# openxrlab/xrslam

Measured on AMD Instinct MI355X. Metric: frames/sec, full per-frame hot path (KLT tracker + sliding-window VI-BA), one sequence per GPU, higher is better.
Workload: dtype u8/i16 images, f32 LK with exact i64 reductions, f64 BA

## Files before the change

xrslam_amd/csrc/ba_chain.hip.h:

```cpp
#pragma once
#include "ba_kernels.hip.h"

namespace xrhip {

constexpr int CHAIN_MAX_NA = 90;
constexpr int CHAIN_MAX_NI = 8;
constexpr int CHAIN_MAX_F = 64;
constexpr int CHAIN_MAX_OBS = 1024;
constexpr int CHAIN_MAX_FREE = 6;
constexpr int CHAIN_THREADS = 256;

#ifdef XRHIP_KPROF
#define CPROF(slot)                                   \
    do {                                              \
        if (threadIdx.x == 0) {                       \
            const long long cp_n = wall_clock64();    \
            s_ctl.prof[slot] += cp_n - cp_t;          \
            cp_t = cp_n;                              \
        }                                             \
    } while (0)
#else
#define CPROF(slot) \
    do {            \
    } while (0)
#endif

struct ChainLayout {
    int sx, cs, Hp, gp, A, scr, sp, D, gs, grad, gn, delta, gt, wJi, wJj, wr, bref, raw, Hv, oc, rec, xch, total;
};
__host__ __device__ __forceinline__ ChainLayout chain_layout(int F, int na, int NI, int nfree, int nobs) {
    ChainLayout L;
    int o = 0;
    auto take = [&](int n) {
        const int r = o;
        o += (n + 1) & ~1;
        return r;
    };
    L.sx = take(16 * F);
    L.cs = take(16 * F);
    L.Hp = take(na * (na + 1) / 2);
    L.gp = take(na);
    L.A = take(na <= CH_NB ? 2 : tl_doubles(na + 1) + 16 * tl_tile_rows(na + 1));
    L.scr = take(NI * IMU_SCR);
    L.sp = take(na);
    L.D = take(na);
    L.gs = take(na);
    L.grad = take(na);
    L.gn = take(na);
    L.delta = take(na);
    L.gt = take(na);
    L.wJi = take(225 * NI);
    L.wJj = take(225 * NI);
    L.wr = take(16 * NI);
    L.bref = take(6 * NI);
    L.raw = take(15 * NI);
    L.Hv = take(28 * nfree);
    L.oc = take(nobs);
    L.rec = take(XRHIP_IMU_DIM * NI);
    L.xch = take(IMU_XCH * NI);
    L.total = o;
    return L;
}

constexpr int CHAIN_VIS_TILE = 4 * 27 * 65;
constexpr int CHAIN_OBS_CACHE = 16;
enum { CHAIN_OPT_TILE = 1, CHAIN_OPT_CACHE = 2 };
__host__ __device__ __forceinline__ int chain_cache_stride(int M) { return (M + 1) & ~1; }

__device__ __forceinline__ double obs_eval_cached(const BaDims &d, const double *oca, int Mp, int o, const double *state, const Ext &cam,
                                                  double sx, double sy, bool want_j, double *rec, const double *ftab, const int *slot_of,
                                                  const double *ctab) {
    const int inf = (int)oca[15 * Mp + o];
    const int ft = inf & 255, fr = (inf >> 8) & 255;
    const bool at = (inf >> 16) & 1, ar = (inf >> 17) & 1;
    if (!at && !ar) {
        if (want_j)
            for (int i = 0; i < OREC; ++i) rec[i] = 0.0;
        return 0.0;
    }
    ObsConst c;
    c.b1 = v3(oca[o], oca[Mp + o], oca[2 * Mp + o]);
    c.b2 = v3(oca[3 * Mp + o], oca[4 * Mp + o], oca[5 * Mp + o]);
    c.y_ref_center = v3(oca[6 * Mp + o], oca[7 * Mp + o], oca[8 * Mp + o]);
    c.x = v3(oca[9 * Mp + o], oca[10 * Mp + o], oca[11 * Mp + o]);
    const V3 zt = v3(oca[12 * Mp + o], oca[13 * Mp + o], oca[14 * Mp + o]);
    double r[2], Jt[12], Jr[12];
#pragma unroll
    for (int i = 0; i < 12; ++i) Jr[i] = 0.0;
    if (!ar) {
        eval_reprojection_tgt(ftab + 12 * slot_of[ft], ctab, c, zt, sx, sy, r, want_j, Jt);
    } else {
        const FState st = load_state(state + 16 * ft), sr = load_state(state + 16 * fr);
        eval_reprojection_cached(st, sr, ar, c, zt, cam, sx, sy, r, want_j, Jt, Jr);
    }
    const double s = r[0] * r[0] + r[1] * r[1];
    if (want_j) {
        const double sc = d.robust ? sqrt(fmax(2.2250738585072014e-308, 1.0 / (1.0 + s))) : 1.0;
#pragma unroll
        for (int i = 0; i < 12; ++i) {
            rec[i] = at ? Jt[i] * sc : 0.0;
            rec[12 + i] = ar ? Jr[i] * sc : 0.0;
        }
        rec[24] = 0.0;
        rec[25] = 0.0;
        rec[26] = r[0] * sc;
        rec[27] = r[1] * sc;
    }
    return d.robust ? 0.5 * log(1.0 + s) : 0.5 * s;
}

struct ChainArgs {
    const TinyArgs *args;
    int seq, max_rounds, opts;
    const double *link_src;
    int link_frame;
};
__global__ __launch_bounds__(CHAIN_THREADS) void kb_chain(Batch<ChainArgs> batch) {
    const TinyArgs *__restrict__ args = batch.e[blockIdx.z].args;
    const int seq = batch.e[blockIdx.z].seq, max_rounds = batch.e[blockIdx.z].max_rounds, opts = batch.e[blockIdx.z].opts;
    const double *link_src = batch.e[blockIdx.z].link_src;
    const int link_frame = batch.e[blockIdx.z].link_src ? batch.e[blockIdx.z].link_frame : -1;
    const BaDims &d = args->d;
    const BaPtrs &p = args->p;
    const Ext &cam = args->cam, &imu = args->imu;
    const double sx_ = args->sx, sy_ = args->sy;
    extern __shared__ double lds[];
    __shared__ double scratch[64];
    __shared__ double Dblk[CH_NB][CH_NB + 1];
    __shared__ double s_vis[4][CHAIN_MAX_FREE][27];
    __shared__ int s_fail;
    __shared__ int s_free[CHAIN_MAX_FREE], s_slot[CHAIN_MAX_F], s_nfree;
    __shared__ double s_ftab[2][CHAIN_MAX_FREE][12], s_ctab[12];
    __shared__ BaCtl s_ctl;
    const int tid = threadIdx.x, lane = tid & 63;
    const bool split = d.NI > 0;
    const bool imu_lane = lane < d.NI;
    const int ostride = split ? 192 : 256;
    const int otid = (!split || tid < 192) ? tid : (1 << 30);
    const int wtid = tid, wave = tid >> 6;
    constexpr bool worker = true;
    constexpr int nt = 256;
    const int F = d.F, n = d.n, na = d.na, NI = d.NI, M = d.M, MR = d.MR;
#ifdef XRHIP_KPROF
    long long cp_t = wall_clock64();
    const long long cp_t0 = cp_t;
#endif

    if (tid < 64) {
        const bool fr = tid < F && p.fix[tid < F ? tid : 0] != 3;
        const unsigned long long m = __ballot(fr);
        const int slot = __popcll(m & ((1ull << tid) - 1ull));
        if (tid < F) s_slot[tid] = (fr && slot < CHAIN_MAX_FREE) ? slot : -1;
        if (fr && slot < CHAIN_MAX_FREE) s_free[slot] = tid;
        if (tid == 0) s_nfree = min(__popcll(m), CHAIN_MAX_FREE);
    } else {
        constexpr unsigned ctl_words = sizeof(BaCtl) / sizeof(long long);
        const long long *src = reinterpret_cast<const long long *>(static_cast<BaCtl *>(p.ctl));
        long long *dst = reinterpret_cast<long long *>(&s_ctl);
        for (unsigned i = tid - 64; i < ctl_words; i += nt - 64) dst[i] = src[i];
    }
    __syncthreads();
    const int nfree = s_nfree;
    const ChainLayout Lo = chain_layout(F, na, NI, nfree, M + MR);
    double *const X = lds + Lo.sx, *const CS = lds + Lo.cs, *const Hp = lds + Lo.Hp, *const gp = lds + Lo.gp;
    double *const A = lds + Lo.A, *const sp = lds + Lo.sp, *const Dg = lds + Lo.D, *const gs = lds + Lo.gs;
    double *const grad = lds + Lo.grad, *const gn = lds + Lo.gn, *const delta = lds + Lo.delta, *const gt = lds + Lo.gt;
    double *const wJi = lds + Lo.wJi, *const wJj = lds + Lo.wJj, *const wr = lds + Lo.wr, *const bref = lds + Lo.bref;
    double *const raw = lds + Lo.raw, *const Hv = lds + Lo.Hv, *const oc = lds + Lo.oc, *const recs = lds + Lo.rec, *const xch = lds + Lo.xch;
    double *const scr = lds + Lo.scr;
    const bool vis_tile = (opts & CHAIN_OPT_TILE) != 0, use_cache = (opts & CHAIN_OPT_CACHE) != 0;
    const int Mp = chain_cache_stride(M);
    double *const oca = lds + Lo.total + (vis_tile ? CHAIN_VIS_TILE : 0);
    BaCtl *const c = &s_ctl;

    int act[4];
#pragma unroll
    for (int m = 0; m < 4; ++m) {
        const int a = tid + nt * m;
        act[m] = (worker && a < n) ? p.act_inv[a] : -1;
    }
    for (int e = wtid; e < 16 * F; e += nt) X[e] = (e >> 4) == link_frame ? link_src[e & 15] : p.state[e];
    for (int e = wtid; e < 6 * NI; e += nt) bref[e] = p.imu_i[e / 6] == link_frame ? link_src[10 + e % 6] : p.bias_ref[e];
    for (int e = wtid; e < XRHIP_IMU_DIM * NI; e += nt) recs[e] = p.imu_data[e];
    for (int e = wtid; e < NI * IMU_SCR; e += nt) scr[e] = 0.0;
    __syncthreads();
    if (tid < nfree) frame_table(load_state(X + 16 * s_free[tid]), s_ftab[0][tid]);
    else if (tid == 64) ext_table(cam, s_ctab);
    if (use_cache) {
        for (int o = wtid; o < M; o += nt) {
            const int ft = p.obs_tgt[o], fr = p.obs_ref[o];
            const bool at = pose_free(p.fix[ft]), ar = pose_free(p.fix[fr]);
            const V3 zt = v3(p.obs_zt[3 * o], p.obs_zt[3 * o + 1], p.obs_zt[3 * o + 2]);
            if (at || ar) {
                const V3 zr = v3(p.obs_zr[3 * o], p.obs_zr[3 * o + 1], p.obs_zr[3 * o + 2]);
                const ObsConst c = reprojection_constants(load_state(X + 16 * fr), p.depth[p.obs_lm[o]], zt, zr, cam);
                oca[o] = c.b1.x; oca[Mp + o] = c.b1.y; oca[2 * Mp + o] = c.b1.z;
                oca[3 * Mp + o] = c.b2.x; oca[4 * Mp + o] = c.b2.y; oca[5 * Mp + o] = c.b2.z;
                oca[6 * Mp + o] = c.y_ref_center.x; oca[7 * Mp + o] = c.y_ref_center.y; oca[8 * Mp + o] = c.y_ref_center.z;
                oca[9 * Mp + o] = c.x.x; oca[10 * Mp + o] = c.x.y; oca[11 * Mp + o] = c.x.z;
                oca[12 * Mp + o] = zt.x; oca[13 * Mp + o] = zt.y; oca[14 * Mp + o] = zt.z;
            }
            oca[15 * Mp + o] = (double)(ft | (fr << 8) | ((int)at << 16) | ((int)ar << 17));
        }
    }
    __syncthreads();
    CPROF(0);

    bool relin = true;
    int mode = 1, st = ST_RUNNING;
    for (int round = 0; round < max_rounds; ++round) {
        if (relin) {
#ifdef XRHIP_KPROF
            const long long pa_t0 = wall_clock64();
#endif
            for (int o = otid; o < M; o += ostride) {
                double rec[OREC];
                const double co = use_cache ? obs_eval_cached(d, oca, Mp, o, X, cam, sx_, sy_, true, rec, &s_ftab[0][0][0], s_slot, s_ctab)
                                            : obs_eval(d, p, o, X, p.depth, cam, sx_, sy_, true, rec);
                oc[o] = co;
#pragma unroll
                for (int i = 0; i < OREC; ++i) p.orec[(size_t)o * OREC + i] = rec[i];
            }
            for (int o = otid; o < MR; o += ostride) {
                double rec[RREC];
                const double co = rot_eval(d, p, o, X, cam, sx_, sy_, true, rec);
                oc[M + o] = co;
#pragma unroll
                for (int i = 0; i < RREC; ++i) p.rrec[(size_t)o * RREC + i] = rec[i];
            }
#ifdef XRHIP_KPROF
            const long long pa_t1 = wall_clock64();
            if (tid == 0) s_ctl.prof[21] += pa_t1 - pa_t0;
#endif
            bool imu_on = false;
            int nfi = 0, nfj = 0;
            if (imu_lane) {
                const int k = lane, fi = p.imu_i[k], fj = p.imu_j[k];
                nfi = p.fix[fi] != 3;
                nfj = p.fix[fj] != 3;
                imu_on = nfi || nfj;
                if (imu_on) {
                    double *rw = scr + k * IMU_SCR;
                    const FState si = load_state(X + 16 * fi), sj = load_state(X + 16 * fj);
                    const ImuRec pre = load_imu(recs + k * XRHIP_IMU_DIM);
                    const V3 bg0 = v3(bref[6 * k], bref[6 * k + 1], bref[6 * k + 2]);
                    const V3 ba0 = v3(bref[6 * k + 3], bref[6 * k + 4], bref[6 * k + 5]);
                    if (wave == 3) {
                        const V3 rq = imu_residual_rq(si, sj, pre, bg0, imu);
                        rw[0] = rq.x;
                        rw[1] = rq.y;
                        rw[2] = rq.z;
                        double *xk = xch + k * IMU_XCH;
                        store33(xk + 45, imu_jac_jrinv(rq));
                        if (nfi) store33(xk + 36, imu_jac_B(rq));
                        imu_residual_rest(si, sj, pre, bg0, ba0, imu, rw);
                    } else if (wave == 0) {
                        imu_raw_jacobians_part(2, si, sj, pre, bg0, ba0, imu, v3(0, 0, 0), rw + 15, rw + 240, nfi, nfj);
                    } else if (wave == 1) {
                        imu_jac_pre(si, sj, pre, bg0, imu, xch + k * IMU_XCH, nfi, nfj);
                    } else {
                        imu_raw_jacobians_part(3, si, sj, pre, bg0, ba0, imu, v3(0, 0, 0), rw + 15, rw + 240, nfi, nfj);
                    }
                }
            }
#ifdef XRHIP_KPROF
            if (tid == 192) atomicAdd((unsigned long long *)&s_ctl.prof[22], (unsigned long long)(wall_clock64() - pa_t1));
            if (tid == 0) atomicAdd((unsigned long long *)&s_ctl.prof[23], (unsigned long long)(wall_clock64() - pa_t1));
#endif
            __syncthreads();
            CPROF(18);
            auto vis_blocks = [&](int idx, int stride) __attribute__((always_inline)) {
                for (int s = 0; s < nfree; ++s) {
                    const int f = s_free[s], pair = f * F + f;
                    const int s0 = p.pair_start[pair], s1 = p.pair_start[pair + 1];
                    double acc[27];
#pragma unroll
                    for (int i = 0; i < 27; ++i) acc[i] = 0.0;
                    for (int it = s0 + idx; it < s1; it += stride) {
                        const int code = p.pair_items[it];
                        const double *rec = p.orec + (size_t)(code >> 1) * OREC + ((code & 1) ? 12 : 0);
                        double j[12];
#pragma unroll
                        for (int i = 0; i < 12; ++i) j[i] = rec[i];
                        const double *rr = p.orec + (size_t)(code >> 1) * OREC + 26;
                        const double r0 = rr[0], r1 = rr[1];
                        int e = 0;
#pragma unroll
                        for (int a = 0; a < 6; ++a) {
#pragma unroll
                            for (int b = a; b < 6; ++b) acc[e++] += j[a] * j[b] + j[6 + a] * j[6 + b];
                            acc[21 + a] += j[a] * r0 + j[6 + a] * r1;
                        }
                    }
                    if (vis_tile) {
                        double *tw = lds + Lo.total + wave * (27 * 65);
#pragma unroll
                        for (int i = 0; i < 27; ++i) tw[i * 65 + lane] = acc[i];
                        wave_sync();
                        const int row = lane < 27 ? lane : lane - 27;
                        double s2 = 0.0;
                        if (lane < 54) {
                            const double *rp = tw + row * 65 + (lane < 27 ? 0 : 32);
#pragma unroll
                            for (int i = 0; i < 32; ++i) s2 += rp[i];
                        }
                        const double hi = __shfl(s2, (lane + 27) & 63);
                        if (lane < 27) s_vis[wave][s][lane] = s2 + hi;
                        wave_sync();
                    } else {
#pragma unroll
                        for (int i = 0; i < 27; ++i) acc[i] = wave_sum(acc[i]);
                        if (lane == 0)
#pragma unroll
                            for (int i = 0; i < 27; ++i) s_vis[wave][s][i] = acc[i];
                    }
                }
            };
            if (split) {
                if (wave >= 2) {
                    vis_blocks(tid - 128, 128);
                } else if (imu_on) {
                    double *rw = scr + lane * IMU_SCR;
                    const double *xk = xch + lane * IMU_XCH;
                    if (wave == 0) imu_jac_finish0(load33(xk + 45), xk, rw + 15, rw + 240, nfi, nfj);
                    else if (wave == 1)
                        imu_jac_finish1(load33(xk + 45), load33(xk + 36), xk, load33(recs + lane * XRHIP_IMU_DIM + 11), rw + 15, nfi);
                }
            } else {
                vis_blocks(tid, nt);
            }
            __syncthreads();
            CPROF(1);
            for (int e = tid; e < 27 * nfree; e += nt) {
                const int s = e / 27, q = e - 27 * s;
                Hv[28 * s + q] = split ? s_vis[2][s][q] + s_vis[3][s][q] : (s_vis[0][s][q] + s_vis[1][s][q]) + (s_vis[2][s][q] + s_vis[3][s][q]);
            }
            for (int k = 0; k < NI; ++k) {
                const double *rw = scr + k * IMU_SCR, *Ji = rw + 15, *Jj = rw + 240;
                const int fi = p.imu_i[k], fj = p.imu_j[k];
                const bool active = !(p.fix[fi] == 3 && p.fix[fj] == 3);
                const double *S = recs + k * XRHIP_IMU_DIM + 56;
                if (wave == (k & 3)) {
                    double cost = 0.0;
                    if (lane < 15) {
                        double s = 0;
                        if (active)
                            for (int j = 0; j < 15; ++j) s += S[15 * lane + j] * rw[j];
                        wr[16 * k + lane] = s;
                        cost = 0.5 * s * s;
                    }
                    cost = wave_sum(cost);
                    if (lane == 0) wr[16 * k + 15] = cost;
                }
                if (wtid < 225) {
                    const int e = wtid, i = e / 15, cc = e - 15 * i;
                    double a = 0, b = 0;
                    if (active) {
                        const bool col_i = cc < 6 ? pose_free(p.fix[fi]) : motion_free(p.fix[fi]);
                        const bool col_j = cc < 6 ? pose_free(p.fix[fj]) : motion_free(p.fix[fj]);
                        if (col_i)
                            for (int j = 0; j < 15; ++j) a += S[15 * i + j] * Ji[15 * j + cc];
                        if (col_j)
                            for (int j = 0; j < 15; ++j) b += S[15 * i + j] * Jj[15 * j + cc];
                    }
                    wJi[225 * k + e] = a;
                    wJj[225 * k + e] = b;
                }
            }
            __syncthreads();
            CPROF(2);
            for (int e = wtid; e < na * (na + 1) / 2 + na; e += nt) {
                int i, j;
                const bool want_g = e >= na * (na + 1) / 2;
                if (want_g) {
                    i = e - na * (na + 1) / 2;
                    j = 0;
                } else {
                    i = (int)((sqrtf(8.0f * e + 1.0f) - 1.0f) * 0.5f);
                    while (i * (i + 1) / 2 > e) --i;
                    while ((i + 1) * (i + 2) / 2 <= e) ++i;
                    j = e - i * (i + 1) / 2;
                }
                const int a = p.act_idx[i], b = p.act_idx[j];
                const int fa = a / 15, ka = a - 15 * fa, fb = b / 15, kb = b - 15 * fb;
                double h = 0.0, g = 0.0;
                if (ka < 6) {
                    const double *hv = Hv + 28 * s_slot[fa];
                    if (!want_g && kb < 6 && fb == fa) {
                        const int lo = ka < kb ? ka : kb, hi = ka < kb ? kb : ka;
                        h += hv[lo * 6 - lo * (lo - 1) / 2 + (hi - lo)];
                    }
                    if (want_g) g += hv[21 + ka];
                    if (ka < 3) {
                        const int s = p.rotf_start[fa], t = p.rotf_start[fa + 1];
                        for (int it = s; it < t; ++it) {
                            const double *rec = p.rrec + (size_t)p.rotf_items[it] * RREC;
                            if (!want_g && fb == fa && kb < 3) h += rec[ka] * rec[kb] + rec[3 + ka] * rec[3 + kb];
                            if (want_g) g += rec[ka] * rec[6] + rec[3 + ka] * rec[7];
                        }
                    }
                }
                for (int side = 0; side < 2; ++side) {
                    const int k = p.imuf[2 * fa + side];
                    if (k < 0) continue;
                    const double *Ja = (side == 0 ? wJj : wJi) + 225 * k;
                    const int fi = p.imu_i[k], fj = p.imu_j[k];
                    if (want_g) {
                        const double *r = wr + 16 * k;
                        for (int q = 0; q < 15; ++q) g += Ja[15 * q + ka] * r[q];
                    } else if (fb == fi || fb == fj) {
                        const double *Jb = (fb == fj ? wJj : wJi) + 225 * k;
                        for (int q = 0; q < 15; ++q) h += Ja[15 * q + ka] * Jb[15 * q + kb];
                    }
                }
                if (want_g) gp[i] = g;
                else Hp[e] = h;
            }
            CPROF(4);
            double cost_part = 0.0;
            for (int o = wtid; o < M; o += nt) cost_part += oc[o];
            for (int o = wtid; o < MR; o += nt) cost_part += oc[M + o];
            for (int k = wtid; k < NI; k += nt) cost_part += wr[16 * k + 15];
            const double ctot = block_sum(cost_part, scratch);
            if (tid == 0) {
                c->x_cost = ctot + 0.0;
                if (c->first) {
                    c->initial_cost = c->x_cost;
                    c->minimum_cost = c->x_cost;
                }
            }
            __syncthreads();
            CPROF(5);
        }
        const bool want_gmax = relin;
        auto gradmax_side = [&]() __attribute__((always_inline)) {
            if (!want_gmax) return;
            double mx = 0;
            if (lane < nfree) {
                const int f = s_free[lane];
                double neg[15], out[16];
                for (int k = 0; k < 15; ++k) {
                    const int i = p.act_inv[15 * f + k];
                    neg[k] = i >= 0 ? -gp[i] : -0.0;
                }
                const double *s = X + 16 * f;
                state_plus(s, neg, pose_free(p.fix[f]), motion_free(p.fix[f]), out);
                for (int k = 0; k < 16; ++k) mx = fmax(mx, fabs(s[k] - out[k]));
            }
#pragma unroll
            for (int off = 32; off > 0; off >>= 1) mx = fmax(mx, __shfl_xor(mx, off));
            if (lane == 0) c->gmax = mx;
        };
        const double mu = c->mu;
        const int first_lin = c->first;
        bool lin_ok = false;
        if (na <= CH_NB) {
            __syncthreads();
            if (wave == 0) {
                const int i = lane;
                const bool on = i < na;
                const double h = on ? Hp[tri_idx(i, i)] : 1.0;
                double spi = on ? sp[i] : 0.0;
                if (first_lin) spi = on ? 1.0 / (1.0 + sqrt(h)) : 0.0;
                const double Dv = sqrt(fmin(fmax(spi * spi * h, 1e-6), 1e32));
                const double gsv = on ? spi * gp[i] : 0.0;
                const double gtv = on ? spi * (gsv / (Dv * Dv)) : 0.0;
                double Xr[CH_NB];
                double t_i = 0.0;
                const double yi = on ? gp[i] * spi : 0.0;
#pragma unroll
                for (int k = 0; k < CH_NB; ++k) {
                    const double spk = lane_bcast(spi, k), gtk = lane_bcast(gtv, k), yk = lane_bcast(yi, k);
                    double v = (k == lane) ? 1.0 : 0.0;
                    if (on && k < na) {
                        const double hik = Hp[k <= i ? tri_idx(i, k) : tri_idx(k, i)];
                        t_i += hik * gtk;
                        v = hik * (spi * spk);
                        if (k == i) v += mu * Dv * Dv;
                    }
                    if (lane >= CH_NB) v = (lane == 2 * CH_NB) ? yk : ((k == lane - CH_NB) ? 1.0 : 0.0);
                    Xr[k] = v;
                }
                if (on) {
                    if (first_lin) sp[i] = spi;
                    Dg[i] = Dv;
                    gs[i] = gsv;
                }
                double qgg = gtv * t_i;
#pragma unroll
                for (int off = 8; off > 0; off >>= 1) qgg += __shfl_xor(qgg, off);
                qgg = lane_bcast(qgg, 0);
                bool ok = diag16_pivot_pairs(Xr, na, lane);
                double xs = 0.0;
#pragma unroll
                for (int cc = 0; cc < CH_NB; ++cc) xs = fma(Xr[cc], lane_bcast(Xr[cc], 2 * CH_NB), xs);
                const double xs_up = __shfl(xs, (lane + CH_NB) & 63);
                const double ya = on ? xs_up : 0.0;
                if (__ballot(on && !isfinite(ya)) != 0ull) ok = false;
                const double gnv = on ? -Dv * ya : 0.0, grv = on ? gsv / Dv : 0.0;
                if (on) {
                    gn[i] = gnv;
                    grad[i] = grv;
                }
                double r6[6] = {grv * grv, on ? (gnv / Dv) * gsv : 0.0, gnv * gnv, grv * grv, gnv * gnv, grv * gnv};
#pragma unroll
                for (int off = 8; off > 0; off >>= 1)
#pragma unroll
                    for (int q = 0; q < 6; ++q) r6[q] += __shfl_xor(r6[q], off);
                if (lane == 0) {
                    if (ok) {
                        c->alpha = r6[0] / qgg;
                        c->q_gg = qgg;
                        c->q_gn = -r6[0] - mu * r6[1];
                        c->q_nn = -r6[1] - mu * r6[2];
                    }
                    c->gnorm = ok ? sqrt(r6[3]) : 0.0;
                    c->gn_norm = ok ? sqrt(r6[4]) : 0.0;
                    c->gd = ok ? r6[5] : 0.0;
                    c->linear_ok = ok ? 1 : 0;
                }
            } else if (wave == 1) {
                gradmax_side();
            } else if (wave == 2 && mode == 1) {
                if (lane < NI) {
                    const double *sti = X + 16 * p.imu_i[lane];
                    for (int q = 0; q < 6; ++q) bref[6 * lane + q] = sti[10 + q];
                }
                double s2 = 0;
                for (int f = lane; f < F; f += 64) {
                    const double *x = X + 16 * f;
                    if (pose_free(p.fix[f]))
                        for (int k = 0; k < 7; ++k) s2 += x[k] * x[k];
                    if (motion_free(p.fix[f]))
                        for (int k = 7; k < 16; ++k) s2 += x[k] * x[k];
                }
                s2 = wave_sum(s2);
                if (lane == 0) {
                    c->x_norm = sqrt(s2);
                    c->first = 0;
                }
            }
            __syncthreads();
            lin_ok = c->linear_ok != 0;
        } else {
            for (int i = wtid; i < na; i += nt) {
                const double h = Hp[i * (i + 1) / 2 + i];
                if (c->first) sp[i] = 1.0 / (1.0 + sqrt(h));
                const double s = sp[i];
                const double Dv = sqrt(fmin(fmax(s * s * h, 1e-6), 1e32));
                Dg[i] = Dv;
                const double gsv = s * gp[i];
                gs[i] = gsv;
                gt[i] = s * (gsv / (Dv * Dv));
            }
            __syncthreads();
            const int nrows = na + 1, Tt = tl_tile_rows(nrows);
            double *yv = A + tl_doubles(nrows);
            tl_clear(A, na, nrows);
            __syncthreads();
            for (int e = wtid; e < na * (na + 1) / 2; e += nt) {
                int i = (int)((sqrtf(8.0f * e + 1.0f) - 1.0f) * 0.5f);
                while (i * (i + 1) / 2 > e) --i;
                while ((i + 1) * (i + 2) / 2 <= e) ++i;
                const int j = e - i * (i + 1) / 2;
                double v = Hp[e] * (sp[i] * sp[j]);
                if (i == j) v += mu * Dg[i] * Dg[i];
                A[tl_idx(i, j)] = v;
            }
            for (int i = wtid; i < na; i += nt) A[tl_idx(na, i)] = gp[i] * sp[i];
            double qacc = 0;
            for (int i = wave; i < na; i += 4) {
                double t = 0;
                for (int j = lane; j < na; j += 64) t += Hp[i >= j ? i * (i + 1) / 2 + j : j * (j + 1) / 2 + i] * gt[j];
                qacc += gt[i] * t;
            }
            const double qgg = block_sum(qacc, scratch);
            CPROF(6);
            lin_ok = tl_chol(A, na, nrows, &Dblk[0][0], &s_fail, nullptr, gradmax_side);
            CPROF(7);
            if (lin_ok) {
                for (int i = wtid; i < 16 * Tt; i += nt) yv[i] = i < na ? A[tl_idx(na, i)] : 0.0;
                __syncthreads();
                tl_trsv_t(A, na, yv);
                int bad = 0;
                for (int i = wtid; i < na; i += nt) {
                    const double ya = yv[i];
                    gn[i] = -Dg[i] * ya;
                    grad[i] = gs[i] / Dg[i];
                    if (!isfinite(ya)) bad = 1;
                }
                if (bad) atomicExch(&s_fail, 1);
                __syncthreads();
                if (s_fail) lin_ok = false;
            }
            __syncthreads();
            if (lin_ok) {
                double r3[3] = {0, 0, 0};
    #pragma unroll
                for (int m = 0; m < 4; ++m) {
                    const int i = act[m];
                    if (i >= 0) {
                        const double g = grad[i], nn = gn[i];
                        r3[0] += g * g;
                        r3[1] += (nn / Dg[i]) * gs[i];
                        r3[2] += nn * nn;
                    }
                }
                block_sum_n<3>(r3, scratch);
                if (tid == 0) {
                    c->alpha = r3[0] / qgg;
                    c->q_gg = qgg;
                    c->q_gn = -r3[0] - mu * r3[1];
                    c->q_nn = -r3[1] - mu * r3[2];
                }
            }
            if (tid == 0) c->linear_ok = lin_ok ? 1 : 0;
            __syncthreads();
            CPROF(8);
            if (mode == 1) {
                for (int k = wtid; k < NI; k += nt) {
                    const double *sti = X + 16 * p.imu_i[k];
                    for (int i = 0; i < 6; ++i) bref[6 * k + i] = sti[10 + i];
                }
                double s2 = 0;
                for (int f = wtid; f < F; f += nt) {
                    const double *x = X + 16 * f;
                    if (pose_free(p.fix[f]))
                        for (int k = 0; k < 7; ++k) s2 += x[k] * x[k];
                    if (motion_free(p.fix[f]))
                        for (int k = 7; k < 16; ++k) s2 += x[k] * x[k];
                }
                s2 = block_sum(s2, scratch);
                if (tid == 0) {
                    c->x_norm = sqrt(s2);
                    c->first = 0;
                }
                __syncthreads();
            }
            {
                double r3[3] = {0, 0, 0};
    #pragma unroll
                for (int m = 0; m < 4; ++m) {
                    const int i = act[m];
                    if (i >= 0 && lin_ok) {
                        r3[0] += grad[i] * grad[i];
                        r3[1] += gn[i] * gn[i];
                        r3[2] += grad[i] * gn[i];
                    }
                }
                block_sum_n<3>(r3, scratch);
                if (tid == 0) {
                    c->gnorm = sqrt(r3[0]);
                    c->gn_norm = sqrt(r3[1]);
                    c->gd = r3[2];
                }
                __syncthreads();
            }
        }
        CPROF(9);
        TrialScalars t;
        trial_load(c, t);
        bool check_gradient = (mode == 1), skip_finalize = (mode == 3);
        bool have_prev = false;
        double prev_ca = 0, prev_cb = 0, prev_mcc = 0, prev_cost = 0, prev_dn2 = 0, prev_sn = 0;
        int accepted = 0;
        while (t.status == ST_RUNNING) {
            trial_begin(t, skip_finalize, check_gradient);
            skip_finalize = false;
            check_gradient = false;
            if (t.status != ST_RUNNING) break;
            double ca, cb, step_norm;
            dogleg_point(t, t.radius, ca, cb, step_norm);
            double mcc, cost, dn2;
            if (have_prev && ca == prev_ca && cb == prev_cb && step_norm >= 0.0) {
                mcc = prev_mcc;
                cost = prev_cost;
                dn2 = prev_dn2;
                step_norm = prev_sn;
            } else {
                double red2[2] = {0, 0};
#pragma unroll
                for (int m = 0; m < 4; ++m) {
                    const int i = act[m];
                    if (i >= 0) {
                        const double v = ca * grad[i] + cb * gn[i];
                        red2[0] += v * v;
                        const double stv = v / Dg[i];
                        red2[1] += stv * gs[i];
                        delta[i] = stv * sp[i];
                    }
                }
                block_sum_n<2>(red2, scratch);
                if (step_norm < 0) step_norm = sqrt(red2[0]);
                mcc = dogleg_model_change(t, ca, cb, red2[1]);
                __syncthreads();
                CPROF(13);
                for (int f = wtid; f < F; f += nt) {
                    double d15[15];
                    for (int k = 0; k < 15; ++k) {
                        const int i = p.act_inv[15 * f + k];
                        d15[k] = i >= 0 ? delta[i] : 0.0;
                    }
                    state_plus(X + 16 * f, d15, pose_free(p.fix[f]), motion_free(p.fix[f]), CS + 16 * f);
                    if (s_slot[f] >= 0) frame_table(load_state(CS + 16 * f), s_ftab[1][s_slot[f]]);
                }
                __syncthreads();
                CPROF(14);
                double red[2] = {0, 0};
                for (int o = otid; o < M; o += ostride)
                    oc[o] = use_cache ? obs_eval_cached(d, oca, Mp, o, CS, cam, sx_, sy_, false, nullptr, &s_ftab[1][0][0], s_slot, s_ctab)
                                      : obs_eval(d, p, o, CS, p.depth, cam, sx_, sy_, false, nullptr);
                for (int o = otid; o < MR; o += ostride) oc[M + o] = rot_eval(d, p, o, CS, cam, sx_, sy_, false, nullptr);
                if (imu_lane && wave >= 2) {
                    const int k = lane;
                    const int fi = p.imu_i[k], fj = p.imu_j[k];
                    double r15[15];
#pragma unroll
                    for (int q = 0; q < 15; ++q) r15[q] = 0.0;
                    if (!(p.fix[fi] == 3 && p.fix[fj] == 3)) {
                        const FState ci = load_state(CS + 16 * fi), cj = load_state(CS + 16 * fj);
                        const ImuRec cpre = load_imu(recs + k * XRHIP_IMU_DIM);
                        const V3 cbg = v3(bref[6 * k], bref[6 * k + 1], bref[6 * k + 2]);
                        const V3 cba = v3(bref[6 * k + 3], bref[6 * k + 4], bref[6 * k + 5]);
                        if (wave == 3) {
                            const V3 rq = imu_residual_rq(ci, cj, cpre, cbg, imu);
                            r15[0] = rq.x;
                            r15[1] = rq.y;
                            r15[2] = rq.z;
                        } else {
                            imu_residual_rest(ci, cj, cpre, cbg, cba, imu, r15);
                        }
                    }
                    if (wave == 3) {
                        for (int q = 0; q < 3; ++q) raw[15 * k + q] = r15[q];
                    } else {
                        for (int q = 3; q < 15; ++q) raw[15 * k + q] = r15[q];
                    }
                }
                __syncthreads();
                CPROF(15);
                for (int o = wtid; o < M; o += nt) red[0] += oc[o];
                for (int o = wtid; o < MR; o += nt) red[0] += oc[M + o];
                for (int it = wtid; it < NI * 15; it += nt) {
                    const int k = it / 15, i = it - 15 * k;
                    const double *S = recs + k * XRHIP_IMU_DIM + 56 + 15 * i;
                    double acc = 0;
#pragma unroll
                    for (int j = 0; j < 15; ++j) acc += S[j] * raw[15 * k + j];
                    red[0] += 0.5 * acc * acc;
                }
                for (int f = wtid; f < F; f += nt) {
                    const double *a = X + 16 * f, *b = CS + 16 * f;
                    double acc = 0;
                    if (pose_free(p.fix[f]))
                        for (int q = 0; q < 7; ++q) acc += (a[q] - b[q]) * (a[q] - b[q]);
                    if (motion_free(p.fix[f]))
                        for (int q = 7; q < 16; ++q) acc += (a[q] - b[q]) * (a[q] - b[q]);
                    red[1] += acc;
                }
                block_sum_n<2>(red, scratch);
                CPROF(16);
                cost = red[0];
                dn2 = red[1];
                have_prev = true;
                prev_ca = ca;
                prev_cb = cb;
                prev_mcc = mcc;
                prev_cost = cost;
                prev_dn2 = dn2;
                prev_sn = step_norm;
            }
            if (trial_decide(t, 0, mcc, cost, dn2, step_norm)) accepted = 1;
        }
        if (accepted) {
            for (int e = wtid; e < 16 * F; e += nt) X[e] = CS[e];
            for (int e = wtid; e < 12 * nfree; e += nt) (&s_ftab[0][0][0])[e] = (&s_ftab[1][0][0])[e];
        }
        if (tid == 0) trial_store(c, t);
        __syncthreads();
        CPROF(10);
#ifdef XRHIP_KPROF
        if (tid == 0) s_ctl.prof[27] += 1;
#endif
        st = t.status;
        if (st == ST_DONE) break;
        if (st == ST_ACCEPTED) {
            relin = true;
            mode = 1;
        } else if (st == ST_RESOLVE || st == ST_RESOLVE_INNER) {
            relin = false;
            mode = (st == ST_RESOLVE) ? 2 : 3;
        } else {
            break;
        }
    }
    for (int e = wtid; e < 16 * F; e += nt) p.state[e] = X[e];
    __syncthreads();
#ifdef XRHIP_KPROF
    if (tid == 0) s_ctl.prof[12] += wall_clock64() - cp_t0;
#endif
    const int fin = (st == ST_DONE) ? ST_DONE : -1;
    if (tid == 0) c->status = fin;
    __syncthreads();
    for (int e = wtid; e < 16 * F; e += nt) p.host_out[e] = X[e];
    {
        constexpr unsigned ctl_words = sizeof(BaCtl) / sizeof(long long);
        const long long *src = reinterpret_cast<const long long *>(&s_ctl);
        long long *dst = reinterpret_cast<long long *>(static_cast<BaCtl *>(p.ctl));
        long long *hst = reinterpret_cast<long long *>(static_cast<BaCtl *>(p.host_ctl));
        for (unsigned i = tid; i < ctl_words; i += nt) {
            const long long v = src[i];
            dst[i] = v;
            hst[i] = v;
        }
    }
    __threadfence_system();
    __syncthreads();
    if (tid == 0) *reinterpret_cast<volatile int *>(static_cast<int *>(p.host_seq)) = seq;
}

}
```

Measured before the change: 1698.

## Rebalance visual block accumulation across all four waves in split mode

In split mode, waves 0-1 previously did only the IMU Jacobian finish while waves 2-3 accumulated all free-frame visual Hessian blocks. Now waves 0-1 join the visual accumulation after their IMU work, taking odd free-frame indices while waves 2-3 take even ones. Results still land in the s_vis rows 2 and 3 that are later summed. The pair_start bounds are also preloaded into shared memory once instead of being read from global memory every round. The cost is that waves 0-1 may still lag behind if the IMU finish is long, and the per-frame split can be uneven when nfree is odd.

```diff
diff --git a/xrslam_amd/csrc/ba_chain.hip.h b/xrslam_amd/csrc/ba_chain.hip.h
--- a/xrslam_amd/csrc/ba_chain.hip.h
+++ b/xrslam_amd/csrc/ba_chain.hip.h
@@ -130,6 +130,7 @@
     __shared__ double s_vis[4][CHAIN_MAX_FREE][27];
     __shared__ int s_fail;
     __shared__ int s_free[CHAIN_MAX_FREE], s_slot[CHAIN_MAX_F], s_nfree;
+    __shared__ int s_pair[2 * CHAIN_MAX_FREE];
     __shared__ double s_ftab[2][CHAIN_MAX_FREE][12], s_ctab[12];
     __shared__ BaCtl s_ctl;
     const int tid = threadIdx.x, lane = tid & 63;
@@ -183,6 +184,7 @@
     for (int e = wtid; e < 6 * NI; e += nt) bref[e] = p.imu_i[e / 6] == link_frame ? link_src[10 + e % 6] : p.bias_ref[e];
     for (int e = wtid; e < XRHIP_IMU_DIM * NI; e += nt) recs[e] = p.imu_data[e];
     for (int e = wtid; e < NI * IMU_SCR; e += nt) scr[e] = 0.0;
+    if (tid >= 128 && tid < 128 + 2 * nfree) s_pair[tid - 128] = p.pair_start[s_free[(tid - 128) >> 1] * (F + 1) + (tid & 1)];
     __syncthreads();
     if (tid < nfree) frame_table(load_state(X + 16 * s_free[tid]), s_ftab[0][tid]);
     else if (tid == 64) ext_table(cam, s_ctab);
@@ -269,10 +271,9 @@
 #endif
             __syncthreads();
             CPROF(18);
-            auto vis_blocks = [&](int idx, int stride) __attribute__((always_inline)) {
-                for (int s = 0; s < nfree; ++s) {
-                    const int f = s_free[s], pair = f * F + f;
-                    const int s0 = p.pair_start[pair], s1 = p.pair_start[pair + 1];
+            auto vis_blocks = [&](int idx, int stride, int sfirst, int sstep, int row_vis) __attribute__((always_inline)) {
+                for (int s = sfirst; s < nfree; s += sstep) {
+                    const int s0 = s_pair[2 * s], s1 = s_pair[2 * s + 1];
                     double acc[27];
 #pragma unroll
                     for (int i = 0; i < 27; ++i) acc[i] = 0.0;
@@ -305,30 +306,37 @@
                             for (int i = 0; i < 32; ++i) s2 += rp[i];
                         }
                         const double hi = __shfl(s2, (lane + 27) & 63);
-                        if (lane < 27) s_vis[wave][s][lane] = s2 + hi;
+                        if (lane < 27) s_vis[row_vis][s][lane] = s2 + hi;
                         wave_sync();
                     } else {
 #pragma unroll
                         for (int i = 0; i < 27; ++i) acc[i] = wave_sum(acc[i]);
                         if (lane == 0)
 #pragma unroll
-                            for (int i = 0; i < 27; ++i) s_vis[wave][s][i] = acc[i];
+                            for (int i = 0; i < 27; ++i) s_vis[row_vis][s][i] = acc[i];
                     }
                 }
             };
+#ifdef XRHIP_KPROF
+            const long long pb_t0 = wall_clock64();
+#endif
             if (split) {
-                if (wave >= 2) {
-                    vis_blocks(tid - 128, 128);
-                } else if (imu_on) {
+                if (wave < 2 && imu_on) {
                     double *rw = scr + lane * IMU_SCR;
                     const double *xk = xch + lane * IMU_XCH;
                     if (wave == 0) imu_jac_finish0(load33(xk + 45), xk, rw + 15, rw + 240, nfi, nfj);
-                    else if (wave == 1)
-                        imu_jac_finish1(load33(xk + 45), load33(xk + 36), xk, load33(recs + lane * XRHIP_IMU_DIM + 11), rw + 15, nfi);
-                }
+                    else imu_jac_finish1(load33(xk + 45), load33(xk + 36), xk, load33(recs + lane * XRHIP_IMU_DIM + 11), rw + 15, nfi);
+                }
+#ifdef XRHIP_KPROF
+                if (lane == 0 && wave < 2) atomicAdd((unsigned long long *)&s_ctl.prof[24 + wave], (unsigned long long)(wall_clock64() - pb_t0));
+#endif
+                vis_blocks((wave & 1) * 64 + lane, 128, wave >= 2 ? 0 : 1, 2, 2 + (wave & 1));
             } else {
-                vis_blocks(tid, nt);
-            }
+                vis_blocks(tid, nt, 0, 1, wave);
+            }
+#ifdef XRHIP_KPROF
+            if (lane == 0 && (wave == 0 || wave == 2)) atomicAdd((unsigned long long *)&s_ctl.prof[wave == 0 ? 28 : 26], (unsigned long long)(wall_clock64() - pb_t0));
+#endif
             __syncthreads();
             CPROF(1);
             for (int e = tid; e < 27 * nfree; e += nt) {
```

Result: slower. 1623 (-4.4%).
